# r9y9/deepvoice3_pytorch

Measured on AMD Instinct MI355X. Metric: mel-frames/sec/node (train step, deepvoice3_ljspeech), higher is better.
Workload: dtype f16x3

## Files before the change

deepvoice3_pytorch_amd/csrc/conv_gemm_bf16x3.hip:

```cpp
#include "conv_common.h"
#include <math.h>
#include <type_traits>

typedef __bf16 bf16x8 __attribute__((ext_vector_type(8)));
typedef __bf16 bf16x2 __attribute__((ext_vector_type(2)));
typedef _Float16 f16x8 __attribute__((ext_vector_type(8)));
typedef _Float16 f16x2 __attribute__((ext_vector_type(2)));
typedef float f32x2 __attribute__((ext_vector_type(2)));


namespace {

constexpr int BKC = 32;
constexpr int KB = 4;
constexpr int HALO_MAX = 64;

__device__ __forceinline__ void split8(const float (&v)[8], bf16x8& hi, bf16x8& lo) {
#pragma unroll
  for (int i = 0; i < 8; i += 2) {
    const f32x2 f = {v[i], v[i + 1]};
    const bf16x2 h = __builtin_convertvector(f, bf16x2);
    const f32x2 r = f - __builtin_convertvector(h, f32x2);
    const bf16x2 l = __builtin_convertvector(r, bf16x2);
    hi[i] = h[0]; hi[i + 1] = h[1];
// ... 560 lines not shown
      const bool f16 = a.d.split_terms == DV3_SPLIT_F16X3, m = a.d.xmask != nullptr;
      if (f16) return m ? launch_x3_m<2, 2, 1, true, 3, 1, false, true, 2>(a, lds, st) : launch_x3_m<2, 2, 1, false, 3, 1, false, true, 2>(a, lds, st);
      return m ? launch_x3_m<2, 2, 1, true, 3, 1, false, false, 2>(a, lds, st) : launch_x3_m<2, 2, 1, false, 3, 1, false, false, 2>(a, lds, st);
    }
  }
  if (a.d.split_terms == DV3_SPLIT_F16X3)
    return a.d.xmask ? launch_x3_m<WM, WN, NI, true, 3, 1, false, true>(a, lds, st) : launch_x3_m<WM, WN, NI, false, 3, 1, false, true>(a, lds, st);
  if (a.d.split_terms == 1)
    return a.d.xmask ? launch_x3_m<WM, WN, NI, true, 1>(a, lds, st) : launch_x3_m<WM, WN, NI, false, 1>(a, lds, st);
  return a.d.xmask ? launch_x3_m<WM, WN, NI, true, 3>(a, lds, st) : launch_x3_m<WM, WN, NI, false, 3>(a, lds, st);
}

const TileCfg* pick_tile_x3(const dv3_conv_desc* d, bool gated, int want_tile) {
  const TileCfg* best = nullptr;
  double best_cost = 0;
  const int64_t ntot = (int64_t)d->B * d->Tout;
  for (const TileCfg& c : kCfgs) {
    if (want_tile && c.id != want_tile) continue;
    if (d->pg && !(c.id == 1 || c.id == 2 || c.id == 8 || c.id == 9)) continue;
    const int BM = c.wm * c.mi * 64, BMH = c.wm * c.mi * 32, BN = c.wn * c.ni * 32;
    const int64_t mt = gated ? dv3_cdiv(d->Cg, BMH) : dv3_cdiv(d->M, BM);
    const int64_t ntl = dv3_cdiv64(ntot, BN);
    const double slots = c.id > 6 ? 256.0 : 512.0;
    const double blocks = (double)mt * ntl;
    const double full = floor(blocks / slots), rem = blocks - slots * full;
    const double rounds = (full + (rem == 0 ? 0.0 : (c.id <= 6 && rem <= 256 ? 0.6 : 1.0))) * (slots / 512.0);
    static const double kRel[10] = {0, 1.0, 1.12, 2.0, 2.2, 1.8, 2.0, 9.9, 0.93, 0.87};
    constexpr int kRel2Percent = 112, kRel8Percent = 86;
    double rel = c.id == 2 ? kRel2Percent * 0.01 : c.id == 8 ? kRel8Percent * 0.01 : kRel[c.id];
    if (d->J == 1 && d->Cin <= 512 && (c.id == 1 || c.id == 2 || c.id == 8 || c.id == 9)) rel = 1.0;
    const double cost = rounds * BM * BN * rel;
    if (!best || cost < best_cost) {
      best = &c;
      best_cost = cost;
    }
  }
  return best;
}

}

int dv3_conv_gemm_pp2_dispatch(const dv3_conv_desc* d, hipStream_t st);

int dv3_conv_gemm_bf16x3_dispatch(const dv3_conv_desc* d, hipStream_t st) {
  const bool gated = d->mode == DV3_EPI_GLU || d->mode == DV3_EPI_HIGHWAY;
  if (d->a_bs != 0 || (d->lda & 3) || d->Tin != d->Tout) return 1;
  if ((d->J - 1) * d->dil > HALO_MAX || d->J * 2 > 32) return 1;
  if ((int64_t)d->B * d->Tout >= (1ll << 30) || (int64_t)d->B * d->x_bs >= (1ll << 30)) return 1;
  if (d->xmask && (int64_t)d->B * d->Cin * d->xmask_rs >= (1ll << 30)) return 1;
  if ((int64_t)d->J * ((d->Cin + 31) / 32 * 4) * d->lda >= (1ll << 27)) return 1;
  const int64_t pp2_tiles = (int64_t)(gated ? dv3_cdiv(d->Cg, 128) : dv3_cdiv(d->M, 256)) * dv3_cdiv64((int64_t)d->B * d->Tout, 256);
  const int pp2_min = dv3_sw(DV3_SW_X3_PP2_MIN_TILES), pp2_sk = dv3_sw(DV3_SW_PP2_SK);
  constexpr int kPp2SkUnitsPerCu = 8;
  const bool sk_fill = d->sk_ws && pp2_sk && (d->mode != DV3_EPI_DGRAD || pp2_sk >= 2) && pp2_min > 0 && pp2_tiles * (d->Cin / 32) >= (int64_t)kPp2SkUnitsPerCu * 256;
  if (d->tile_hint == 30 || (pp2_min > 0 && d->tile_hint == 0 && (pp2_tiles >= pp2_min || sk_fill))) {
    const int rc = dv3_conv_gemm_pp2_dispatch(d, st);
    if (rc != 1) return rc;
    if (d->tile_hint == 30) return 1;
  }
  const TileCfg* best = pick_tile_x3(d, gated, d->tile_hint > 20 ? d->tile_hint - 20 : 0);
  if (!best) return 1;
  constexpr int kKsMaxBlocks = 256, kKsMinSteps = 8;
  bool ks_ok = false;
  const int ks_form = dv3_sw(DV3_SW_X3_KS);
  if (ks_form && d->split_terms != 1 && (d->tile_hint == 0 || d->tile_hint == 22)) {
    const int64_t nb2 = (int64_t)(gated ? dv3_cdiv(d->Cg, 64) : dv3_cdiv(d->M, 128)) * dv3_cdiv64((int64_t)d->B * d->Tout, 64);
    const int nch = (d->Cin + 31) / 32;
    const int ksteps = nch * d->J;
    ks_ok = nch >= 2 && (ks_form == 2 || (ksteps >= kKsMinSteps && nb2 <= (ksteps >= 16 ? kKsMaxBlocks : kKsMaxBlocks * 5 / 8)));
    if (ks_ok && d->tile_hint == 0 && (best->id == 4 || best->id == 6)) best = &kCfgs[1];
  }
  const int BM = best->wm * best->mi * 64, BMH = best->wm * best->mi * 32, BN = best->wn * best->ni * 32;
  const int BNH = BN + (d->J - 1) * d->dil;
  const size_t lds = (size_t)(2 * 2 * KB * BM + 2 * 2 * KB * BNH) * 16;
  if (lds > 160 * 1024) return 1;
  ConvArgs a;
  a.d = *d;
  a.a_scalar = 0;
  a.wide = dv3_sw(DV3_SW_X3_WIDE);
  a.prio = dv3_sw(DV3_SW_X3_PRIO);
  a.range_ctr = d->split_terms == DV3_SPLIT_F16X3 ? dv3_range_ctr() : nullptr;
  a.kp = (d->Cin + 31) / 32 * 32;
  a.m_tiles = gated ? dv3_cdiv(d->Cg, BMH) : dv3_cdiv(d->M, BM);
  a.n_tiles = (int)dv3_cdiv64((int64_t)d->B * d->Tout, BN);
  const int64_t nb = (int64_t)a.m_tiles * a.n_tiles;
  DV3_REQUIRE(nb < (1ll << 31), "conv_gemm: grid too large");
  a.n_blocks = (int)nb;
  a.ks = (ks_ok && best->id == 2 && 2 * lds <= 160 * 1024) ? 2 : 0;
  g_dv3_last_conv = (d->split_terms == 1 ? 4000 : d->split_terms == DV3_SPLIT_F16X3 ? 5000 : 3000) + best->id * 10 +
                    ((best->id >= 8 && dv3_sw(DV3_SW_X3_PINGPONG)) ? 1 : 0) + (a.ks == 2 ? 2 : 0);
  if (d->pg) {
    if (d->xmask || d->split_terms == DV3_SPLIT_F16X3 || d->split_terms == 1) return 1;
    g_dv3_last_conv += 600;
    switch (best->id) {
      case 1: return launch_x3_m<2, 2, 2, false, 3, 1, false, false, 1, true>(a, lds, st);
      case 2: return a.ks == 2 ? launch_x3_m<2, 2, 1, false, 3, 1, false, false, 2, true>(a, lds, st)
                               : launch_x3_m<2, 2, 1, false, 3, 1, false, false, 1, true>(a, lds, st);
      case 8: return launch_x3_m<4, 2, 2, false, 3, 1, true, false, 1, true>(a, lds, st);
      case 9: return launch_x3_m<2, 4, 2, false, 3, 1, true, false, 1, true>(a, lds, st);
    }
    return 1;
  }
  switch (best->id) {
    case 1: return launch_x3<2, 2, 2>(a, lds, st);
    case 2: return launch_x3<2, 2, 1>(a, lds, st);
    case 3: return launch_x3<4, 1, 1>(a, lds, st);
    case 4: return launch_x3<2, 1, 1>(a, lds, st);
    case 5: return launch_x3<1, 2, 2>(a, lds, st);
// ... 22 lines not shown
```

deepvoice3_pytorch_amd/csrc/conv_gemm_pp2.hip:

```cpp
#include "conv_common.h"
#include <math.h>
#include <type_traits>

typedef __bf16 bf16x8 __attribute__((ext_vector_type(8)));
typedef __bf16 bf16x2 __attribute__((ext_vector_type(2)));
typedef _Float16 f16x8 __attribute__((ext_vector_type(8)));
typedef float f32x2 __attribute__((ext_vector_type(2)));

namespace {

constexpr int BKC = 32, KB = 4, HALO_MAX = 64;
constexpr int BM = 256, BMH = 128, BN = 256, NT = 512, MI = 2, NI = 2, WN = 4;
constexpr int JT = 3;
constexpr int AU = KB * BM / NT;
constexpr int XI = (KB * (BN + HALO_MAX) + NT - 1) / NT;
static_assert(AU == 2, "one panel unit per k16 phase");

__device__ __forceinline__ void pp2_split8(const float (&v)[8], bf16x8& hi, bf16x8& lo) {
#pragma unroll
  for (int i = 0; i < 8; i += 2) {
    const f32x2 f = {v[i], v[i + 1]};
    const bf16x2 h = __builtin_convertvector(f, bf16x2);
    const f32x2 r = f - __builtin_convertvector(h, f32x2);
    const bf16x2 l = __builtin_convertvector(r, bf16x2);
    hi[i] = h[0]; hi[i + 1] = h[1];
    lo[i] = l[0]; lo[i + 1] = l[1];
  }
}
template <bool F16>
__device__ __forceinline__ f32x16 pp2_mma(const bf16x8& a, const bf16x8& b, const f32x16& c) {
  if constexpr (F16)
    return __builtin_amdgcn_mfma_f32_32x32x16_f16(__builtin_bit_cast(f16x8, a), __builtin_bit_cast(f16x8, b), c, 0, 0, 0);
  else
    return __builtin_amdgcn_mfma_f32_32x32x16_bf16(a, b, c, 0, 0, 0);
}
template <bool OPAQUE>
__device__ __forceinline__ const ConvArgs* dv3_opaque_args(const ConvArgs* a) {
  if constexpr (OPAQUE) {
    int off = 0;
    asm volatile("" : "+s"(off));
    return reinterpret_cast<const ConvArgs*>(reinterpret_cast<const char*>(a) + off);
  } else {
    return a;
  }
}
template <typename T>
__device__ __forceinline__ T pp2_ldg(const void* base, uint32_t byte_off) {
  return *reinterpret_cast<const T*>(reinterpret_cast<const char*>(base) + byte_off);
}

template <bool MASK, bool F16, bool SK = false, int ORD = 0, bool PW = false, bool FG = false>
__global__ __launch_bounds__(NT) void conv_gemm_pp2_kernel(const ConvArgs args) {
  static_assert(!PW || (!MASK && !F16 && !SK), "pair words: the unmasked bf16-pair tile-per-workgroup form");
  static_assert(!FG || (!MASK && !F16 && !SK), "fused gate backward: the unmasked bf16-pair tile-per-workgroup form");
  const dv3_conv_desc& p = args.d;
  extern __shared__ __attribute__((aligned(16))) unsigned char smem_raw[];
  constexpr int J = JT;
  bf16x8* const As = reinterpret_cast<bf16x8*>(smem_raw);
  bf16x8* const Xs = As + 2 * 2 * KB * BM;

  int pid_ = dv3_xcd_remap(blockIdx.x, args.n_blocks);
  if constexpr (SK) {
    const int q = 1 << args.sk_qshift;
    pid_ = (pid_ & ~(q - 1)) + (q - 1 - (pid_ & (q - 1)));
  }
  const int pid = pid_;
  const int nchunks = p.Cin / BKC;
  int seg_u = 0, seg_end = 0, sk_base = 0, sk_rem = 0, sk_g0 = 0;
  if constexpr (SK) {
    const int grp = pid >> args.sk_qshift, slot = pid & ((1 << args.sk_qshift) - 1);
    const bool big = grp < args.sk_tr;
    sk_base = big ? args.sk_base : args.sk_base2;
    sk_rem = big ? args.sk_rem : args.sk_rem2;
    sk_g0 = (grp * args.sk_tg + min(grp, args.sk_tr)) << args.sk_shift;
    seg_u = sk_g0 + slot * sk_base + min(slot, sk_rem);
    seg_end = seg_u + sk_base + (slot < sk_rem ? 1 : 0);
  }
  constexpr bool WIDE_GLU = (ORD & 32) != 0;
  int tid_ = threadIdx.x;
  const int wave_s = __builtin_amdgcn_readfirstlane(tid_ >> 6);
  do {
  const ConvArgs& A = *dv3_opaque_args<SK>(&args);
  const dv3_conv_desc& p = A.d;
  const int dil = p.dil;
  const int BNH = BN + (J - 1) * dil;
  const int xbuf = 2 * KB * BNH;
  if constexpr (SK) {
    int lane_;
    asm volatile("v_mbcnt_lo_u32_b32 %0, -1, 0\n\tv_mbcnt_hi_u32_b32 %0, -1, %0" : "=v"(lane_));
    tid_ = wave_s * 64 + lane_;
  }
  const int tid = tid_;
  const int lane = tid & 63;
  const int wave = __builtin_amdgcn_readfirstlane(tid >> 6);
  const int wm = wave / WN, wn = wave % WN;
  const int l31 = lane & 31, lhi = lane >> 5;
  int tile_ = pid, c0_ = 0, c1_ = nchunks;
  if constexpr (SK) {
    tile_ = seg_u >> A.sk_shift;
    c0_ = seg_u - tile_ * nchunks;
    c1_ = min(nchunks, c0_ + (seg_end - seg_u));
  }
  const int tile = tile_, c0 = SK ? c0_ : 0, c1 = SK ? c1_ : nchunks;
  const int mt = SK ? (tile & (A.m_tiles - 1)) : tile % A.m_tiles;
  const int nt = SK ? (tile >> A.sk_mshift) : tile / A.m_tiles;
  const int n0 = nt * BN;

  const bool gated = (p.mode == DV3_EPI_GLU || p.mode == DV3_EPI_HIGHWAY);
  int h0b, h1b;
  if (gated) {
    h0b = mt * BMH; h1b = p.a_half + mt * BMH;
  } else {
    h0b = mt * BM; h1b = mt * BM + BMH;
  }

  const int Cin = p.Cin, T = p.Tout, lda = p.lda, B = p.B;
  const int Ntot = B * T;
  const int k8_total = A.kp >> 3;
  const bf16x8* __restrict__ Wh = reinterpret_cast<const bf16x8*>(p.a_split);
  const int64_t plane = (int64_t)J * k8_total * lda;
  const float xscale = F16 ? (float)(1 << DV3_F16_ACT_SHIFT) : 1.0f;
  const float dscale = p.drop_scale * xscale;

  uint32_t vbits = 0;
#pragma unroll
  for (int ni = 0; ni < NI; ++ni) {
    const int n = n0 + wn * (NI * 32) + ni * 32 + l31;
    const int bc = n / T, tc = n - bc * T;
    for (int j = 0; j < J; ++j) {
      const int ts = tc + j * dil - p.padL;
      if (n < Ntot && ts >= 0 && ts < T) vbits |= 1u << (j * NI + ni);
    }
  }
  uint32_t need = 0;
  for (int j = 0; j < J; ++j) {
    const uint32_t all = ((1u << NI) - 1u) << (j * NI);
    if (!__all((vbits & all) == all)) need |= 1u << j;
  }
  need = __builtin_amdgcn_readfirstlane(need);

  uint32_t xoff[XI];
  const int n_items = KB * BNH;
  const uint32_t x_rsb = (uint32_t)p.x_rs * 4u;
  const uint32_t c8p = (uint32_t)((Cin + 31) / 32 * 4);
#pragma unroll
  for (int i = 0; i < XI; ++i) {
    const int idx = tid + i * NT;
    const int k8 = idx / BNH, q = idx - k8 * BNH;
    const int f = n0 - p.padL + q;
    int bf = 0, tf = 0;
    if (idx < n_items && f >= 0 && f < Ntot) {
      bf = f / T;
      tf = f - bf * T;
    }
    const int xk8 = k8 < KB ? k8 * 8 : 0;
    xoff[i] = ((uint32_t)bf * (uint32_t)p.x_bs + (uint32_t)tf) * 4u + (uint32_t)xk8 * x_rsb;
  }
  constexpr bool LEAN = (ORD & 2) != 0 && !SK;
  uint32_t aoff_r[2] = {0u, 0u};
  auto aoff_of = [&](int u) -> uint32_t {
    if constexpr (LEAN) return aoff_r[u];
    int t_ = tid;
    asm volatile("" : "+v"(t_));
    const int idx = t_ + u * NT;
    const int col = idx % BM, k8 = idx / BM;
    const bool hi_half = col >= BMH;
    const int gcol = (hi_half ? h1b : h0b) + (col - (hi_half ? BMH : 0));
    return (uint32_t)(k8 * lda + (gcol < lda ? gcol : 0)) * 16u;
  };

  if constexpr (LEAN) {
#pragma unroll
    for (int u = 0; u < 2; ++u) {
      const int idx = tid + u * NT;
      const int col = idx % BM, k8 = idx / BM;
      const bool hi_half = col >= BMH;
      const int gcol = (hi_half ? h1b : h0b) + (col - (hi_half ? BMH : 0));
      aoff_r[u] = (uint32_t)(k8 * lda + (gcol < lda ? gcol : 0)) * 16u;
    }
  }

  bf16x8 ra[2];
  float rx[XI][8];
  uint32_t rk[MASK ? XI : 1];

  auto load_A_unit = [&](int chunk, int j, auto uc) {
    constexpr int u = decltype(uc)::value;
    const bf16x8* srch = Wh + (int64_t)(j * k8_total + chunk * KB) * lda;
    const uint32_t ao = aoff_of(u);
    ra[0] = pp2_ldg<bf16x8>(srch, ao);
    ra[1] = pp2_ldg<bf16x8>(srch + plane, ao);
  };
  auto write_A_unit = [&](int buf, auto uc) {
    constexpr int u = decltype(uc)::value;
    bf16x8* dst = As + buf * (2 * KB * BM);
    dst[tid + u * NT] = ra[0];
    dst[KB * BM + tid + u * NT] = ra[1];
  };
  auto load_X_half = [&](int chunk, auto ic, auto hc) {
    constexpr int i = decltype(ic)::value, h = decltype(hc)::value;
    const char* xb = reinterpret_cast<const char*>(p.x) + (int64_t)(chunk * BKC) * x_rsb;
    uint32_t rs = x_rsb;
    asm volatile("" : "+s"(rs));
#pragma unroll
    for (int e = 4 * h; e < 4 * h + 4; ++e) {
      uint32_t er = (uint32_t)e * rs;
      if constexpr (SK) {
        if (e == 0) { er = 0; asm volatile("" : "+s"(er)); }
      }
      rx[i][e] = pp2_ldg<float>(xb, xoff[i] + er);
    }
    if constexpr (MASK && h == 1) {
      int t_ = tid;
      asm volatile("" : "+v"(t_));
      const int idx = t_ + i * NT;
      const int k8 = idx / BNH, q = idx - k8 * BNH;
      const int f = n0 - p.padL + q;
      int bf = 0, tf = 0;
      if (idx < n_items && f >= 0 && f < Ntot) {
        bf = f / T;
        tf = f - bf * T;
      }
      const uint32_t mo = ((uint32_t)bf * c8p + (uint32_t)(k8 < KB ? k8 : 0)) * (uint32_t)T + (uint32_t)tf;
      rk[i] = (uint32_t)pp2_ldg<uint8_t>(p.xmask_c8 + (int64_t)chunk * 4 * T, mo);
    }
  };
  auto write_X_item = [&](int buf, auto ic) {
    constexpr int i = decltype(ic)::value;
    bf16x8* dst = Xs + buf * xbuf;
    const int idx = tid + i * NT;
    float v[8];
    uint32_t keep = MASK ? rk[i] : 0u;
    if constexpr (MASK && SK) asm("" : "+v"(keep));
#pragma unroll
    for (int e = 0; e < 8; ++e) {
      v[e] = rx[i][e];
      if constexpr (MASK) v[e] *= ((keep >> e) & 1u) ? dscale : 0.f;
      else if (F16) v[e] *= xscale;
    }
    bf16x8 hi, lo;
    if constexpr (PW) {
      uint32_t w[8];
#pragma unroll
      for (int e = 0; e < 8; ++e) w[e] = __float_as_uint(rx[i][e]);
      dv3_pair_units(w, hi, lo);
    } else if constexpr (F16 && LEAN) {
      const float m0 = fmaxf(fmaxf(fabsf(v[0]), fabsf(v[1])), fabsf(v[2]));
      const float m1 = fmaxf(fmaxf(fabsf(v[3]), fabsf(v[4])), fabsf(v[5]));
      const float m = fmaxf(fmaxf(m0, m1), fmaxf(fabsf(v[6]), fabsf(v[7])));
      const bool bad = !(m <= 65504.f);
      if (__builtin_expect(__any(bad), 0)) {
        dv3_note_range(A.range_ctr, dv3_split8_f16(v, hi, lo));
      } else {
        f16x8 h8, l8;
#pragma unroll
        for (int e = 0; e < 8; e += 2) {
          const f32x2 f = {v[e], v[e + 1]};
          typedef _Float16 f16x2_ __attribute__((ext_vector_type(2)));
          const f16x2_ h = __builtin_convertvector(f, f16x2_);
          h8[e] = h[0]; h8[e + 1] = h[1];
          if constexpr ((ORD & 8) != 0) {
            uint32_t l2 = 0u;
            const uint32_t h2 = __builtin_bit_cast(uint32_t, h);
            asm("v_fma_mixlo_f16 %0, %1, -1.0, %2 op_sel:[0,0,0] op_sel_hi:[1,0,0]" : "+v"(l2) : "v"(h2), "v"(v[e]));
            asm("v_fma_mixhi_f16 %0, %1, -1.0, %2 op_sel:[1,0,0] op_sel_hi:[1,0,0]" : "+v"(l2) : "v"(h2), "v"(v[e + 1]));
            const f16x2_ l = __builtin_bit_cast(f16x2_, l2);
            l8[e] = l[0]; l8[e + 1] = l[1];
          } else {
            l8[e] = (_Float16)(v[e] - (float)h[0]);
            l8[e + 1] = (_Float16)(v[e + 1] - (float)h[1]);
          }
        }
        hi = __builtin_bit_cast(bf16x8, h8);
        lo = __builtin_bit_cast(bf16x8, l8);
      }
    } else if constexpr (F16) dv3_note_range(A.range_ctr, dv3_split8_f16(v, hi, lo)); else pp2_split8(v, hi, lo);
    if (idx < n_items) {
      dst[idx] = hi;
      dst[KB * BNH + idx] = lo;
    }
  };
  uint32_t sbad = 0;
  auto write_X_item_nb = [&](int buf, auto ic) {
    constexpr int i = decltype(ic)::value;
    bf16x8* dst = Xs + buf * xbuf;
    const int idx = tid + i * NT;
    float v[8];
    const uint32_t keep = MASK ? rk[i] : 0u;
#pragma unroll
    for (int e = 0; e < 8; ++e) {
      v[e] = rx[i][e];
      if constexpr (MASK) {
        v[e] *= ((keep >> e) & 1u) ? dscale : 0.f;
        asm("" : "+v"(v[e]));
      } else if (F16) v[e] *= xscale;
    }
    bf16x8 hi, lo;
    if constexpr (PW) {
      uint32_t w[8];
#pragma unroll
      for (int e = 0; e < 8; ++e) w[e] = __float_as_uint(rx[i][e]);
      dv3_pair_units(w, hi, lo);
    } else if constexpr (F16) {
      const bool bad = dv3_split8_f16(v, hi, lo);
      sbad += (uint32_t)__builtin_popcountll(__ballot(bad));
    } else {
      pp2_split8(v, hi, lo);
    }
    const int spare = 2 * xbuf - buf * xbuf;
    const bool live = i < 2 || idx < n_items;
    dst[live ? idx : spare] = hi;
    dst[live ? KB * BNH + idx : spare + 1] = lo;
  };
  using U0 = std::integral_constant<int, 0>;
  using U1 = std::integral_constant<int, 1>;
  using U2 = std::integral_constant<int, 2>;
  constexpr bool CVC = (ORD & 64) != 0 && !SK;
  static_assert(XI == 3 && JT == 3, "three activation items per thread, one per tap's pair of k16 phases");

  f32x16 acc[MI][2][NI];
  float zero_ = 0.f;
  if constexpr (SK) asm volatile("" : "+v"(zero_));
#pragma unroll
  for (int mi = 0; mi < MI; ++mi)
#pragma unroll
    for (int h = 0; h < 2; ++h)
#pragma unroll
      for (int ni = 0; ni < NI; ++ni)
#pragma unroll
        for (int r = 0; r < 16; ++r) acc[mi][h][ni][r] = zero_;

  const int a_off = wm * (MI * 32) + l31;
  const int x_off = wn * (NI * 32) + l31;

  load_A_unit(c0, 0, U0{});
  write_A_unit(0, U0{});
  load_A_unit(c0, 0, U1{});
  load_X_half(c0, U0{}, U0{}); load_X_half(c0, U0{}, U1{});
  load_X_half(c0, U1{}, U0{}); load_X_half(c0, U1{}, U1{});
  load_X_half(c0, U2{}, U0{}); load_X_half(c0, U2{}, U1{});
  write_A_unit(0, U1{});
  write_X_item(0, U0{});
  write_X_item(0, U1{});
  write_X_item(0, U2{});
  __syncthreads();
  {
    const int cp = min(c0 + 1, c1 - 1);
    load_A_unit(c0, 1, U0{});
    load_X_half(cp, U0{}, U0{});
    load_X_half(cp, U0{}, U1{});
    load_X_half(cp, U1{}, U0{}); load_X_half(cp, U1{}, U1{});
    load_X_half(cp, U2{}, U0{});
    if constexpr (!CVC) load_X_half(cp, U2{}, U1{});
  }

  const bool pf_on = (ORD & 4) != 0 && !SK && gated && p.r != nullptr;
  const int late = wave >> 2;
  if (late) __syncthreads();
  for (int c = c0; c < c1; ++c) {
    const int cr = c - c0;
    const bf16x8* XsH = Xs + (cr & 1) * xbuf;
    const bf16x8* XsL = XsH + KB * BNH;
    const int cx = min(c + 2, c1 - 1);
    const bool last_chunk = c + 1 == c1;
#pragma unroll
    for (int q = 0; q < 2 * JT; ++q) {
      constexpr int dummy = 0; (void)dummy;
      const int j = q >> 1, s = q & 1;
      const int cur = (cr * JT + j) & 1;
      const bf16x8* AsH = As + cur * (2 * KB * BM);
      const bf16x8* AsL = AsH + KB * BM;
      const bool fix = (need >> j) & 1u;
      bf16x8 ah[MI][2], al[MI][2], bh[NI], bl[NI];
      auto read_frags = [&](bool do_a, bool do_b) {
        const int k8 = 2 * s + lhi;
        if (do_a) {
          const int ai = k8 * BM + a_off;
#pragma unroll
          for (int mi = 0; mi < MI; ++mi) {
            ah[mi][0] = AsH[ai + mi * 32];
            ah[mi][1] = AsH[ai + mi * 32 + BMH];
            al[mi][0] = AsL[ai + mi * 32];
            al[mi][1] = AsL[ai + mi * 32 + BMH];
          }
        }
        if (do_b) {
          const int xi = k8 * BNH + x_off + j * dil;
#pragma unroll
          for (int ni = 0; ni < NI; ++ni) {
            bh[ni] = XsH[xi + ni * 32];
            bl[ni] = XsL[xi + ni * 32];
          }
        }
      };
      auto fix_frags = [&]() {
        const int k8 = 2 * s + lhi; (void)k8;
        if (fix) {
          const bf16x8 zero8 = {0, 0, 0, 0, 0, 0, 0, 0};
#pragma unroll
          for (int ni = 0; ni < NI; ++ni) {
            const bool ok = (vbits >> (j * NI + ni)) & 1u;
            bh[ni] = ok ? bh[ni] : zero8;
            bl[ni] = ok ? bl[ni] : zero8;
          }
        }
      };
      if constexpr ((ORD & 1) != 0) {
        read_frags(true, (ORD & 16) == 0);
        __builtin_amdgcn_sched_barrier(0);
      }
      {
        int jn = j + 1, cn = c;
        if (jn >= JT) { jn = 0; cn = c + 1; }
        int j2 = jn + 1, c2 = cn;
        if (j2 >= JT) { j2 = 0; c2 = cn + 1; }
        if (cn >= c1) { cn = c; jn = j; }
        if (c2 >= c1) { c2 = c; j2 = j; }
        if (s == 0) {
          write_A_unit(cur ^ 1, U0{});
          load_A_unit(cn, jn, U1{});
        } else {
          write_A_unit(cur ^ 1, U1{});
          load_A_unit(c2, j2, U0{});
        }
        if constexpr (CVC) {
          const int cx1 = min(c + 1, c1 - 1);
          if (q == 0) load_X_half(cx1, U2{}, U1{});
          if (q == 1) load_X_half(cx, U0{}, U0{});
          if (q == 2) load_X_half(cx, U0{}, U1{});
          if (q == 3) load_X_half(cx, U1{}, U0{});
          if (q == 4) load_X_half(cx, U1{}, U1{});
          if (q == 5) load_X_half(cx, U2{}, U0{});
        } else {
        if (q == 0) { write_X_item((cr + 1) & 1, U0{}); load_X_half(cx, U0{}, U0{}); }
        if (q == 1) { load_X_half(cx, U0{}, U1{}); }
        if (q == 2) { write_X_item((cr + 1) & 1, U1{}); load_X_half(cx, U1{}, U0{}); }
        if (q == 3) { load_X_half(cx, U1{}, U1{}); }
        if (q == 4) { write_X_item((cr + 1) & 1, U2{}); load_X_half(cx, U2{}, U0{}); }
        if (q == 5) { load_X_half(cx, U2{}, U1{}); }
        }
        if constexpr ((ORD & 4) != 0 && !SK) {
          if ((q == 1 || q == 3) && last_chunk && pf_on) {
            typedef const __attribute__((address_space(1))) void* gptr;
            typedef __attribute__((address_space(3))) void* lptr;
            unsigned char* strip = smem_raw + (size_t)(2 * 2 * KB * BM + 2 * xbuf) * 16 + wave * 256;
            int t_ = tid;
            asm volatile("" : "+v"(t_));
            const int row = t_ >> 2, col = (t_ & 3) * 64 + (q >> 1) * 32;
            const int ch = min(mt * BMH + row, p.Cg - 1);
            const int n = min(n0 + col, Ntot - 1);
            const int bb = n / T, tt = n - bb * T;
            const uint32_t po = ((uint32_t)bb * (uint32_t)p.r_bs + (uint32_t)ch * (uint32_t)p.r_rs + (uint32_t)tt) * 4u;
            __builtin_amdgcn_global_load_lds((gptr)(reinterpret_cast<const char*>(p.r) + po), (lptr)strip, 4, 0, 0);
          }
        }
      }
      __builtin_amdgcn_sched_barrier(0);
      if constexpr ((ORD & 1) == 0) read_frags(true, true);
      else if constexpr ((ORD & 16) != 0) read_frags(false, true);
      fix_frags();
      __syncthreads();
      __builtin_amdgcn_sched_barrier(0);
#pragma unroll
      for (int mi = 0; mi < MI; ++mi)
#pragma unroll
        for (int ni = 0; ni < NI; ++ni) {
          acc[mi][0][ni] = pp2_mma<F16>(al[mi][0], bh[ni], acc[mi][0][ni]);
          acc[mi][1][ni] = pp2_mma<F16>(al[mi][1], bh[ni], acc[mi][1][ni]);
        }
#pragma unroll
      for (int mi = 0; mi < MI; ++mi)
#pragma unroll
        for (int ni = 0; ni < NI; ++ni) {
          acc[mi][0][ni] = pp2_mma<F16>(ah[mi][0], bl[ni], acc[mi][0][ni]);
          acc[mi][1][ni] = pp2_mma<F16>(ah[mi][1], bl[ni], acc[mi][1][ni]);
        }
#pragma unroll
      for (int mi = 0; mi < MI; ++mi)
#pragma unroll
        for (int ni = 0; ni < NI; ++ni) {
          acc[mi][0][ni] = pp2_mma<F16>(ah[mi][0], bh[ni], acc[mi][0][ni]);
          acc[mi][1][ni] = pp2_mma<F16>(ah[mi][1], bh[ni], acc[mi][1][ni]);
        }
      if constexpr (CVC) {
        if (q == 0) write_X_item_nb((cr + 1) & 1, U0{});
        if (q == 2) write_X_item_nb((cr + 1) & 1, U1{});
        if (q == 4) write_X_item_nb((cr + 1) & 1, U2{});
        if ((q & 1) == 0) {
#pragma unroll
          for (int m = 0; m < 22; ++m) {
            __builtin_amdgcn_sched_group_barrier(0x008, 1, 0);
            __builtin_amdgcn_sched_group_barrier(0x002, 3, 0);
          }
          __builtin_amdgcn_sched_group_barrier(0x008, 1, 0);
          __builtin_amdgcn_sched_group_barrier(0x200, 1, 0);
          __builtin_amdgcn_sched_group_barrier(0x008, 1, 0);
          __builtin_amdgcn_sched_group_barrier(0x200, 1, 0);
        }
      }
      __builtin_amdgcn_sched_barrier(0);
      if (!(last_chunk && q == 2 * JT - 1) || !late) __syncthreads();
    }
  }
  if constexpr (CVC && F16) {
    if (sbad != 0 && lane == 0 && A.range_ctr) atomicAdd(A.range_ctr, sbad);
  }

  bool run_tail = true;
  if constexpr (SK) {
    constexpr int ACC = MI * 2 * NI * 16;
    float* const ws = A.sk_ws;
    int* const flags = A.sk_flags;
    if (c0 != 0) {
      char* dst = reinterpret_cast<char*>(ws) + ((size_t)pid * (ACC * NT) + (size_t)tid * 4) * 4;
#pragma unroll
      for (int mi = 0; mi < MI; ++mi)
#pragma unroll
        for (int h = 0; h < 2; ++h)
#pragma unroll
          for (int ni = 0; ni < NI; ++ni)
#pragma unroll
            for (int r4 = 0; r4 < 4; ++r4) {
              typedef float f32x4_ __attribute__((ext_vector_type(4)));
              const f32x4_ v4 = {acc[mi][h][ni][r4 * 4], acc[mi][h][ni][r4 * 4 + 1], acc[mi][h][ni][r4 * 4 + 2], acc[mi][h][ni][r4 * 4 + 3]};
              const char* d4 = dst + (size_t)((((mi * 2 + h) * NI + ni) * 4 + r4) * NT) * 16;
              asm volatile("global_store_dwordx4 %0, %1, off sc0 sc1" ::"v"(d4), "v"(v4) : "memory");
            }
      asm volatile("s_waitcnt vmcnt(0)" ::: "memory");
      __builtin_amdgcn_fence(__ATOMIC_RELEASE, "workgroup");
      __syncthreads();
      if (tid == 0) __hip_atomic_store(flags + pid, 1, __ATOMIC_RELAXED, __HIP_MEMORY_SCOPE_AGENT);
      run_tail = false;
    } else if (c1 < nchunks) {
      const int qm = (1 << A.sk_qshift) - 1;
      for (int w2 = pid + 1; (w2 & qm) != 0; ++w2) {
        const int s2 = sk_g0 + (w2 & qm) * sk_base + min(w2 & qm, sk_rem);
        if (s2 >= (tile + 1) * nchunks) break;
        if (tid == 0)
          while (__hip_atomic_load(flags + w2, __ATOMIC_RELAXED, __HIP_MEMORY_SCOPE_AGENT) == 0) __builtin_amdgcn_s_sleep(8);
        __syncthreads();
        __builtin_amdgcn_fence(__ATOMIC_ACQUIRE, "workgroup");
        const char* src = reinterpret_cast<const char*>(ws) + ((size_t)w2 * (ACC * NT) + (size_t)tid * 4) * 4;
        typedef const __attribute__((address_space(1))) void* gptr_;
        typedef __attribute__((address_space(3))) void* lptr_;
#pragma unroll
        for (int half = 0; half < 2; ++half) {
#pragma unroll
          for (int jq = 0; jq < 16; ++jq) {
            const int qg = half * 16 + jq;
            __builtin_amdgcn_global_load_lds((gptr_)(src + (size_t)(qg * NT) * 16), (lptr_)(smem_raw + (jq * NT + wave * 64) * 16), 16, 0, 17);
          }
          asm volatile("s_waitcnt vmcnt(0)" ::: "memory");
#pragma unroll
          for (int jq = 0; jq < 16; ++jq) {
// ... 38 lines not shown
      bcol[ni] = n / T;
      tcol[ni] = n - bcol[ni] * T;
    }
    if constexpr (FG) {
      const int nw0 = n0e + wn * (NI * 32);
      if (dv3_wide_gate_ok(pt, AT.wide)) {
        float* wl = reinterpret_cast<float*>(smem_raw) + wave * (DV3_WIDE_LDS / 4);
#pragma unroll
        for (int mi = 0; mi < MI; ++mi) {
          const int row0 = wm * (MI * 32) + mi * 32;
          conv_epilogue_wide_block_gate<BM, BMH>(pt, acc[mi][0], mt, row0, 0, lane, nw0, Ntot, wl);
          conv_epilogue_wide_block_gate<BM, BMH>(pt, acc[mi][1], mt, row0, 1, lane, nw0, Ntot, wl);
        }
      } else {
        conv_epilogue_dgrad_gate<BM, BMH, NI>(pt, acc[0], mt, wm * (MI * 32), lhi, l31, bcol, tcol, okc, nw0 >> 5);
        conv_epilogue_dgrad_gate<BM, BMH, NI>(pt, acc[1], mt, wm * (MI * 32) + 32, lhi, l31, bcol, tcol, okc, nw0 >> 5);
      }
    } else
    if (dv3_wide_epilogue_ok(pt, AT.wide)) {
      float* wl = reinterpret_cast<float*>(smem_raw) + wave * (DV3_WIDE_LDS / 4);
      const int nw0 = n0e + wn * (NI * 32);
#pragma unroll
      for (int mi = 0; mi < MI; ++mi) {
        const int row0 = wm * (MI * 32) + mi * 32;
        conv_epilogue_wide_block<BM, BMH>(pt, acc[mi][0], mt, row0, 0, lane, nw0, Ntot, wl);
        conv_epilogue_wide_block<BM, BMH>(pt, acc[mi][1], mt, row0, 1, lane, nw0, Ntot, wl);
      }
    } else if (WIDE_GLU && dv3_wide_glu_ok(pt)) {
      const int nw0 = n0e + wn * (NI * 32);
      conv_epilogue_glu_wide<BMH, NI>(pt, acc[0], mt, wm * (MI * 32), lane, nw0, Ntot);
      conv_epilogue_glu_wide<BMH, NI>(pt, acc[1], mt, wm * (MI * 32) + 32, lane, nw0, Ntot);
    } else {
      bool interior = false;
      if constexpr (!SK)
        interior = AT.fast_tail && gated && !pt.spk && pt.store_mode == DV3_STORE_BCT &&
                   mt * BMH + wm * (MI * 32) + MI * 32 <= pt.Cg && n0e + wn * (NI * 32) + NI * 32 <= Ntot;
      if (!SK && interior) {
        conv_epilogue_glu_interior<BMH, NI>(pt, acc[0], mt, wm * (MI * 32), lhi, bcol, tcol);
        conv_epilogue_glu_interior<BMH, NI>(pt, acc[1], mt, wm * (MI * 32) + 32, lhi, bcol, tcol);
      } else {
        conv_epilogue<BM, BMH, NI, false>(pt, acc[0], gated, mt, wm * (MI * 32), lhi, bcol, tcol, okc);
        conv_epilogue<BM, BMH, NI, false>(pt, acc[1], gated, mt, wm * (MI * 32) + 32, lhi, bcol, tcol, okc);
      }
    }
  }
  if constexpr (SK) {
    seg_u += c1 - c0;
    __syncthreads();
  }
  } while (SK && seg_u < seg_end);
}

#ifndef DV3_PP2_ISA_ONLY
template <bool MASK, bool F16, bool SK = false, int ORD = 0, bool PW = false, bool FG = false>
int launch_pp2(const ConvArgs& a, size_t lds, hipStream_t st) {
  if ((ORD & 4) != 0 && lds + 8 * 256 > 160 * 1024) return launch_pp2<MASK, F16, SK, (ORD & ~4), PW, FG>(a, lds, st);
  static bool attr_set = false;
  if (!attr_set) {
    hipError_t e = hipFuncSetAttribute((const void*)conv_gemm_pp2_kernel<MASK, F16, SK, ORD, PW, FG>,
                                       hipFuncAttributeMaxDynamicSharedMemorySize, 160 * 1024);
    if (e != hipSuccess) {
      dv3_set_error("conv_gemm_pp2: hipFuncSetAttribute: %s", hipGetErrorString(e));
      return DV3_ELAUNCH;
    }
    attr_set = true;
  }
  if ((ORD & 4) != 0) lds += 8 * 256;
  else if ((ORD & 64) != 0) lds += 32;
  hipLaunchKernelGGL((conv_gemm_pp2_kernel<MASK, F16, SK, ORD, PW, FG>), dim3(a.n_blocks), dim3(NT), lds, st, a);
  return dv3_check_launch("conv_gemm_pp2");
}

#endif
}

#ifndef DV3_PP2_ISA_ONLY

constexpr int kSkOverheadChunks = 2, kSkGainPercent = 80;
static int pp2_cu_count() {
  static int n = 0;
  if (!n) {
    int dev = 0, v = 0;
    if (hipGetDevice(&dev) == hipSuccess && hipDeviceGetAttribute(&v, hipDeviceAttributeMultiprocessorCount, dev) == hipSuccess && v > 0) n = v;
    else n = 256;
  }
  return n;
}
int64_t dv3_pp2_sk_ws_bytes() { return (int64_t)pp2_cu_count() * (128 * NT * 4 + 64); }
extern "C" int dv3_conv_streamk_ws_bytes(void) { return (int)dv3_pp2_sk_ws_bytes(); }

int dv3_conv_gemm_pp2_dispatch(const dv3_conv_desc* d, hipStream_t st) {
  if (d->split_terms == 1 || !d->a_split) return 1;
  if (d->xmask && !d->xmask_c8) return 1;
  if (d->J != JT || (d->J - 1) * d->dil > HALO_MAX || (d->Cin & 31)) return 1;
  if (d->a_bs != 0 || (d->lda & 3) || d->Tin != d->Tout) return 1;
  const bool gated = d->mode == DV3_EPI_GLU || d->mode == DV3_EPI_HIGHWAY;
  const bool f16 = d->split_terms == DV3_SPLIT_F16X3;
  const int BNH = BN + (d->J - 1) * d->dil;
  const size_t lds = (size_t)(2 * 2 * KB * BM + 2 * 2 * KB * BNH) * 16;
  if (lds > 160 * 1024) return 1;
  ConvArgs a;
  a.d = *d;
  a.a_scalar = 0;
  a.wide = dv3_sw(DV3_SW_X3_WIDE);
  a.fast_tail = dv3_sw(DV3_SW_PP2_FAST_TAIL);
  a.range_ctr = f16 ? dv3_range_ctr() : nullptr;
  a.kp = (d->Cin + 31) / 32 * 32;
  a.m_tiles = gated ? dv3_cdiv(d->Cg, BMH) : dv3_cdiv(d->M, BM);
  a.n_tiles = (int)dv3_cdiv64((int64_t)d->B * d->Tout, BN);
  const int64_t nb = (int64_t)a.m_tiles * a.n_tiles;
  DV3_REQUIRE(nb < (1ll << 31), "conv_gemm: grid too large");
  a.n_blocks = (int)nb;
  g_dv3_last_conv = (f16 ? 5000 : 3000) + 100 + 1;
  const bool mask = d->xmask_c8 != nullptr;
  if (d->x_pair || d->pg) {
    if (mask || f16) return 1;
    g_dv3_last_conv += (d->x_pair ? 5 : 0) + (d->pg ? 10 : 0);
    if (d->pg) return d->x_pair ? launch_pp2<false, false, false, 81, true, true>(a, lds, st)
                                : launch_pp2<false, false, false, 81, false, true>(a, lds, st);
    return launch_pp2<false, false, false, 81, true>(a, lds, st);
  }
  {
    const int P = pp2_cu_count(), S = d->Cin / BKC;
    const int64_t units = nb * S;
    const int sk_form = dv3_sw(DV3_SW_PP2_SK);
    const int64_t dp = dv3_cdiv64(nb, P) * S, sk = dv3_cdiv64(units, P) + kSkOverheadChunks;
    const bool ws_ok = d->sk_ws && d->sk_ws_bytes >= dv3_pp2_sk_ws_bytes() && units < (1ll << 30);
    const bool dir_ok = d->mode != DV3_EPI_DGRAD || sk_form >= 2;
    const int q = P / 8;
    const bool grp_ok = (P % 8) == 0 && q > 0 && (q & (q - 1)) == 0 && nb >= 8;
    if (ws_ok && dir_ok && grp_ok && sk_form && (S & (S - 1)) == 0 && (a.m_tiles & (a.m_tiles - 1)) == 0 && units >= 2 * P && (sk_form == 2 || sk * 100 < dp * kSkGainPercent)) {
      a.sk_units = (int)units;
      a.sk_tg = (int)(nb / 8);
      a.sk_tr = (int)(nb % 8);
      a.sk_qshift = __builtin_ctz((unsigned)q);
      const int64_t ub = (int64_t)(a.sk_tg + 1) * S, us = (int64_t)a.sk_tg * S;
      a.sk_base = (int)(ub / q);
      a.sk_rem = (int)(ub % q);
      a.sk_base2 = (int)(us / q);
      a.sk_rem2 = (int)(us % q);
      a.sk_shift = __builtin_ctz((unsigned)S);
      a.sk_mshift = __builtin_ctz((unsigned)a.m_tiles);
      a.n_blocks = P;
      a.sk_flags = reinterpret_cast<int*>(d->sk_ws);
      a.sk_ws = reinterpret_cast<float*>(reinterpret_cast<char*>(d->sk_ws) + (size_t)P * 64);
      g_dv3_last_conv += 1;
      const size_t lds_sk = lds;
      if (f16) return mask ? launch_pp2<true, true, true>(a, lds_sk, st) : launch_pp2<false, true, true>(a, lds_sk, st);
      return mask ? launch_pp2<true, false, true>(a, lds_sk, st) : launch_pp2<false, false, true>(a, lds_sk, st);
    }
  }
  {
    const int o = mask ? (f16 ? dv3_sw(DV3_SW_PP2_ORD_M) : 0) : dv3_sw(DV3_SW_PP2_ORD_U);
#define DV3_PP2_ORD_SHIP(oo) \
    if (o == oo) { \
      if (f16) return mask ? launch_pp2<true, true, false, oo>(a, lds, st) : launch_pp2<false, true, false, oo>(a, lds, st); \
      return mask ? launch_pp2<true, false, false, oo>(a, lds, st) : launch_pp2<false, false, false, oo>(a, lds, st); \
    }
    DV3_PP2_ORD_SHIP(17) DV3_PP2_ORD_SHIP(81)
#undef DV3_PP2_ORD_SHIP
  }
  if (f16) return mask ? launch_pp2<true, true>(a, lds, st) : launch_pp2<false, true>(a, lds, st);
  return mask ? launch_pp2<true, false>(a, lds, st) : launch_pp2<false, false>(a, lds, st);
}
#else
namespace {
template __global__ void conv_gemm_pp2_kernel<DV3_PP2_ISA_MASK, true, false, DV3_PP2_ISA_ORD>(const ConvArgs);
// ... 3 lines not shown
```

Baseline: 3.767 million.

## Extend pp2 256x256 conv GEMM kernel to single-tap (1x1) convolutions

Adds a JN template parameter so the large-tile pp2 split-precision GEMM kernel can run one-tap convolutions. Channel counts that are not multiples of 32 are handled by zero-filling the K tail. The activation pipeline is restructured to two items per thread with a separate schedule, and an FMA-based lo-term split is used on the masked bf16 path. The dispatcher routes J==1 convs to pp2 using a tile-count and K-step rule, which adds kernel variants and risks poor occupancy on small shapes.

```diff
diff --git a/deepvoice3_pytorch_amd/csrc/conv_gemm_bf16x3.hip b/deepvoice3_pytorch_amd/csrc/conv_gemm_bf16x3.hip
--- a/deepvoice3_pytorch_amd/csrc/conv_gemm_bf16x3.hip
+++ b/deepvoice3_pytorch_amd/csrc/conv_gemm_bf16x3.hip
@@ -636,8 +636,18 @@
   const int64_t pp2_tiles = (int64_t)(gated ? dv3_cdiv(d->Cg, 128) : dv3_cdiv(d->M, 256)) * dv3_cdiv64((int64_t)d->B * d->Tout, 256);
   const int pp2_min = dv3_sw(DV3_SW_X3_PP2_MIN_TILES), pp2_sk = dv3_sw(DV3_SW_PP2_SK);
   constexpr int kPp2SkUnitsPerCu = 8;
-  const bool sk_fill = d->sk_ws && pp2_sk && (d->mode != DV3_EPI_DGRAD || pp2_sk >= 2) && pp2_min > 0 && pp2_tiles * (d->Cin / 32) >= (int64_t)kPp2SkUnitsPerCu * 256;
-  if (d->tile_hint == 30 || (pp2_min > 0 && d->tile_hint == 0 && (pp2_tiles >= pp2_min || sk_fill))) {
+  const bool sk_fill = d->J != 1 && d->sk_ws && pp2_sk && (d->mode != DV3_EPI_DGRAD || pp2_sk >= 2) && pp2_min > 0 && pp2_tiles * (d->Cin / 32) >= (int64_t)kPp2SkUnitsPerCu * 256;
+  constexpr int kJ1MinTiles = 192, kJ1FwdMinKsteps = 8, kJ1DgradMinKsteps = 4, kJ1CuCount = 256;
+  bool pp2_rule = pp2_min > 0 && (pp2_tiles >= pp2_min || sk_fill);
+  if (d->J == 1) {
+    const bool dgrad = d->mode == DV3_EPI_DGRAD;
+    const int ksteps = (d->Cin + 31) / 32;
+    const int fwd_k = kJ1FwdMinKsteps * (pp2_tiles > kJ1CuCount ? 2 : 1);
+    const bool measured = pp2_tiles >= kJ1MinTiles && ksteps >= (dgrad ? kJ1DgradMinKsteps : fwd_k) &&
+                          2 * dv3_cdiv(d->M, 256) == dv3_cdiv(d->M, 128);
+    pp2_rule = pp2_min == 1 || (pp2_min > 0 && measured);
+  }
+  if (d->tile_hint == 30 || (d->tile_hint == 0 && pp2_rule)) {
     const int rc = dv3_conv_gemm_pp2_dispatch(d, st);
     if (rc != 1) return rc;
     if (d->tile_hint == 30) return 1;
diff --git a/deepvoice3_pytorch_amd/csrc/conv_gemm_pp2.hip b/deepvoice3_pytorch_amd/csrc/conv_gemm_pp2.hip
--- a/deepvoice3_pytorch_amd/csrc/conv_gemm_pp2.hip
+++ b/deepvoice3_pytorch_amd/csrc/conv_gemm_pp2.hip
@@ -13,7 +13,8 @@
 constexpr int BM = 256, BMH = 128, BN = 256, NT = 512, MI = 2, NI = 2, WN = 4;
 constexpr int JT = 3;
 constexpr int AU = KB * BM / NT;
-constexpr int XI = (KB * (BN + HALO_MAX) + NT - 1) / NT;
+constexpr int XI3 = (KB * (BN + HALO_MAX) + NT - 1) / NT;
+constexpr int XI1 = KB * BN / NT;
 static_assert(AU == 2, "one panel unit per k16 phase");
 
 __device__ __forceinline__ void pp2_split8(const float (&v)[8], bf16x8& hi, bf16x8& lo) {
@@ -49,13 +50,15 @@
   return *reinterpret_cast<const T*>(reinterpret_cast<const char*>(base) + byte_off);
 }
 
-template <bool MASK, bool F16, bool SK = false, int ORD = 0, bool PW = false, bool FG = false>
+template <bool MASK, bool F16, bool SK = false, int ORD = 0, bool PW = false, bool FG = false, int JN = JT>
 __global__ __launch_bounds__(NT) void conv_gemm_pp2_kernel(const ConvArgs args) {
   static_assert(!PW || (!MASK && !F16 && !SK), "pair words: the unmasked bf16-pair tile-per-workgroup form");
   static_assert(!FG || (!MASK && !F16 && !SK), "fused gate backward: the unmasked bf16-pair tile-per-workgroup form");
+  static_assert(JN == JT || (JN == 1 && !SK && !FG && (ORD & (4 | 32)) == 0), "one tap: tile per workgroup, plain tails");
+  constexpr int XI = JN == 1 ? XI1 : XI3;
   const dv3_conv_desc& p = args.d;
   extern __shared__ __attribute__((aligned(16))) unsigned char smem_raw[];
-  constexpr int J = JT;
+  constexpr int J = JN;
   bf16x8* const As = reinterpret_cast<bf16x8*>(smem_raw);
   bf16x8* const Xs = As + 2 * 2 * KB * BM;
 
@@ -65,7 +68,7 @@
     pid_ = (pid_ & ~(q - 1)) + (q - 1 - (pid_ & (q - 1)));
   }
   const int pid = pid_;
-  const int nchunks = p.Cin / BKC;
+  const int nchunks = JN == 1 ? (p.Cin + BKC - 1) / BKC : p.Cin / BKC;
   int seg_u = 0, seg_end = 0, sk_base = 0, sk_rem = 0, sk_g0 = 0;
   if constexpr (SK) {
     const int grp = pid >> args.sk_qshift, slot = pid & ((1 << args.sk_qshift) - 1);
@@ -83,7 +86,7 @@
   const ConvArgs& A = *dv3_opaque_args<SK>(&args);
   const dv3_conv_desc& p = A.d;
   const int dil = p.dil;
-  const int BNH = BN + (J - 1) * dil;
+  const int BNH = JN == 1 ? BN : BN + (J - 1) * dil;
   const int xbuf = 2 * KB * BNH;
   if constexpr (SK) {
     int lane_;
@@ -106,7 +109,7 @@
   const int nt = SK ? (tile >> A.sk_mshift) : tile / A.m_tiles;
   const int n0 = nt * BN;
 
-  const bool gated = (p.mode == DV3_EPI_GLU || p.mode == DV3_EPI_HIGHWAY);
+  const bool gated = JN == 3 && (p.mode == DV3_EPI_GLU || p.mode == DV3_EPI_HIGHWAY);
   int h0b, h1b;
   if (gated) {
     h0b = mt * BMH; h1b = p.a_half + mt * BMH;
@@ -202,9 +205,15 @@
     const char* xb = reinterpret_cast<const char*>(p.x) + (int64_t)(chunk * BKC) * x_rsb;
     uint32_t rs = x_rsb;
     asm volatile("" : "+s"(rs));
+    int lim = BKC, kr = 0;
+    if constexpr (JN == 1) {
+      lim = Cin - chunk * BKC;
+      kr = (2 * i + (wave >> 2)) * 8;
+    }
 #pragma unroll
     for (int e = 4 * h; e < 4 * h + 4; ++e) {
       uint32_t er = (uint32_t)e * rs;
+      if constexpr (JN == 1) er = kr + e < lim ? er : 0u - (uint32_t)kr * rs;
       if constexpr (SK) {
         if (e == 0) { er = 0; asm volatile("" : "+s"(er)); }
       }
@@ -225,10 +234,15 @@
       rk[i] = (uint32_t)pp2_ldg<uint8_t>(p.xmask_c8 + (int64_t)chunk * 4 * T, mo);
     }
   };
-  auto write_X_item = [&](int buf, auto ic) {
+  auto write_X_item = [&](int buf, int cw, auto ic) {
     constexpr int i = decltype(ic)::value;
     bf16x8* dst = Xs + buf * xbuf;
     const int idx = tid + i * NT;
+    if constexpr (JN == 1) {
+      const int lim = Cin - cw * BKC, kr = (2 * i + (wave >> 2)) * 8;
+#pragma unroll
+      for (int e = 0; e < 8; ++e) rx[i][e] = kr + e < lim ? rx[i][e] : 0.f;
+    }
     float v[8];
     uint32_t keep = MASK ? rk[i] : 0u;
     if constexpr (MASK && SK) asm("" : "+v"(keep));
@@ -239,6 +253,14 @@
       else if (F16) v[e] *= xscale;
     }
     bf16x8 hi, lo;
+    if constexpr (JN == 1 && MASK && !F16) {
+#pragma unroll
+      for (int e = 0; e < 8; ++e) {
+        const __bf16 h = (__bf16)v[e];
+        hi[e] = h;
+        lo[e] = (__bf16)__builtin_fmaf(rx[i][e], ((keep >> e) & 1u) ? dscale : 0.f, -(float)h);
+      }
+    } else
     if constexpr (PW) {
       uint32_t w[8];
 #pragma unroll
@@ -281,21 +303,38 @@
     }
   };
   uint32_t sbad = 0;
-  auto write_X_item_nb = [&](int buf, auto ic) {
+  auto write_X_item_nb = [&](int buf, int cw, auto ic) {
     constexpr int i = decltype(ic)::value;
     bf16x8* dst = Xs + buf * xbuf;
     const int idx = tid + i * NT;
+    if constexpr (JN == 1) {
+      const int lim = Cin - cw * BKC, kr = (2 * i + (wave >> 2)) * 8;
+#pragma unroll
+      for (int e = 0; e < 8; ++e) rx[i][e] = kr + e < lim ? rx[i][e] : 0.f;
+    }
     float v[8];
     const uint32_t keep = MASK ? rk[i] : 0u;
+    constexpr bool FMA_LO = JN == 1 && MASK && !F16;
+    float ksel[FMA_LO ? 8 : 1];
 #pragma unroll
     for (int e = 0; e < 8; ++e) {
       v[e] = rx[i][e];
       if constexpr (MASK) {
-        v[e] *= ((keep >> e) & 1u) ? dscale : 0.f;
+        const float sel = ((keep >> e) & 1u) ? dscale : 0.f;
+        v[e] *= sel;
         asm("" : "+v"(v[e]));
+        if constexpr (FMA_LO) ksel[e] = sel;
       } else if (F16) v[e] *= xscale;
     }
     bf16x8 hi, lo;
+    if constexpr (FMA_LO) {
+#pragma unroll
+      for (int e = 0; e < 8; ++e) {
+        const __bf16 h = (__bf16)v[e];
+        hi[e] = h;
+        lo[e] = (__bf16)__builtin_fmaf(rx[i][e], ksel[e], -(float)h);
+      }
+    } else
     if constexpr (PW) {
       uint32_t w[8];
 #pragma unroll
@@ -316,7 +355,7 @@
   using U1 = std::integral_constant<int, 1>;
   using U2 = std::integral_constant<int, 2>;
   constexpr bool CVC = (ORD & 64) != 0 && !SK;
-  static_assert(XI == 3 && JT == 3, "three activation items per thread, one per tap's pair of k16 phases");
+  static_assert((XI == 3 && JN == 3) || (XI == 2 && JN == 1), "three taps: one activation item per tap's pair of k16 phases; one tap: one per phase");
 
   f32x16 acc[MI][2][NI];
   float zero_ = 0.f;
@@ -338,20 +377,26 @@
   load_A_unit(c0, 0, U1{});
   load_X_half(c0, U0{}, U0{}); load_X_half(c0, U0{}, U1{});
   load_X_half(c0, U1{}, U0{}); load_X_half(c0, U1{}, U1{});
-  load_X_half(c0, U2{}, U0{}); load_X_half(c0, U2{}, U1{});
+  if constexpr (JN == 3) { load_X_half(c0, U2{}, U0{}); load_X_half(c0, U2{}, U1{}); }
   write_A_unit(0, U1{});
-  write_X_item(0, U0{});
-  write_X_item(0, U1{});
-  write_X_item(0, U2{});
+  write_X_item(0, c0, U0{});
+  write_X_item(0, c0, U1{});
+  if constexpr (JN == 3) write_X_item(0, c0, U2{});
   __syncthreads();
   {
     const int cp = min(c0 + 1, c1 - 1);
+    if constexpr (JN == 3) {
     load_A_unit(c0, 1, U0{});
     load_X_half(cp, U0{}, U0{});
     load_X_half(cp, U0{}, U1{});
     load_X_half(cp, U1{}, U0{}); load_X_half(cp, U1{}, U1{});
     load_X_half(cp, U2{}, U0{});
     if constexpr (!CVC) load_X_half(cp, U2{}, U1{});
+    } else {
+      load_A_unit(cp, 0, U0{});
+      load_X_half(cp, U0{}, U0{}); load_X_half(cp, U0{}, U1{});
+      load_X_half(cp, U1{}, U0{}); load_X_half(cp, U1{}, U1{});
+    }
   }
 
   const bool pf_on = (ORD & 4) != 0 && !SK && gated && p.r != nullptr;
@@ -364,10 +409,10 @@
     const int cx = min(c + 2, c1 - 1);
     const bool last_chunk = c + 1 == c1;
 #pragma unroll
-    for (int q = 0; q < 2 * JT; ++q) {
+    for (int q = 0; q < 2 * J; ++q) {
       constexpr int dummy = 0; (void)dummy;
       const int j = q >> 1, s = q & 1;
-      const int cur = (cr * JT + j) & 1;
+      const int cur = (cr * J + j) & 1;
       const bf16x8* AsH = As + cur * (2 * KB * BM);
       const bf16x8* AsL = AsH + KB * BM;
       const bool fix = (need >> j) & 1u;
@@ -411,9 +456,9 @@
       }
       {
         int jn = j + 1, cn = c;
-        if (jn >= JT) { jn = 0; cn = c + 1; }
+        if (jn >= J) { jn = 0; cn = c + 1; }
         int j2 = jn + 1, c2 = cn;
-        if (j2 >= JT) { j2 = 0; c2 = cn + 1; }
+        if (j2 >= J) { j2 = 0; c2 = cn + 1; }
         if (cn >= c1) { cn = c; jn = j; }
         if (c2 >= c1) { c2 = c; j2 = j; }
         if (s == 0) {
@@ -423,6 +468,18 @@
           write_A_unit(cur ^ 1, U1{});
           load_A_unit(c2, j2, U0{});
         }
+        if constexpr (JN == 1) {
+          if constexpr (CVC) {
+            if (q == 1) {
+              load_X_half(cx, U0{}, U0{}); load_X_half(cx, U0{}, U1{});
+              load_X_half(cx, U1{}, U0{}); load_X_half(cx, U1{}, U1{});
+            }
+          } else {
+            const int cw = min(c + 1, c1 - 1);
+            if (q == 0) { write_X_item((cr + 1) & 1, cw, U0{}); load_X_half(cx, U0{}, U0{}); load_X_half(cx, U0{}, U1{}); }
+            if (q == 1) { write_X_item((cr + 1) & 1, cw, U1{}); load_X_half(cx, U1{}, U0{}); load_X_half(cx, U1{}, U1{}); }
+          }
+        } else
         if constexpr (CVC) {
           const int cx1 = min(c + 1, c1 - 1);
           if (q == 0) load_X_half(cx1, U2{}, U1{});
@@ -432,11 +489,11 @@
           if (q == 4) load_X_half(cx, U1{}, U1{});
           if (q == 5) load_X_half(cx, U2{}, U0{});
         } else {
-        if (q == 0) { write_X_item((cr + 1) & 1, U0{}); load_X_half(cx, U0{}, U0{}); }
+        if (q == 0) { write_X_item((cr + 1) & 1, c, U0{}); load_X_half(cx, U0{}, U0{}); }
         if (q == 1) { load_X_half(cx, U0{}, U1{}); }
-        if (q == 2) { write_X_item((cr + 1) & 1, U1{}); load_X_half(cx, U1{}, U0{}); }
+        if (q == 2) { write_X_item((cr + 1) & 1, c, U1{}); load_X_half(cx, U1{}, U0{}); }
         if (q == 3) { load_X_half(cx, U1{}, U1{}); }
-        if (q == 4) { write_X_item((cr + 1) & 1, U2{}); load_X_half(cx, U2{}, U0{}); }
+        if (q == 4) { write_X_item((cr + 1) & 1, c, U2{}); load_X_half(cx, U2{}, U0{}); }
         if (q == 5) { load_X_half(cx, U2{}, U1{}); }
         }
         if constexpr ((ORD & 4) != 0 && !SK) {
@@ -483,9 +540,25 @@
           acc[mi][1][ni] = pp2_mma<F16>(ah[mi][1], bh[ni], acc[mi][1][ni]);
         }
       if constexpr (CVC) {
-        if (q == 0) write_X_item_nb((cr + 1) & 1, U0{});
-        if (q == 2) write_X_item_nb((cr + 1) & 1, U1{});
-        if (q == 4) write_X_item_nb((cr + 1) & 1, U2{});
+        if constexpr (JN == 1) {
+          if (q == 0) {
+            const int cw = min(c + 1, c1 - 1);
+            write_X_item_nb((cr + 1) & 1, cw, U0{});
+            write_X_item_nb((cr + 1) & 1, cw, U1{});
+#pragma unroll
+            for (int m = 0; m < 22; ++m) {
+              __builtin_amdgcn_sched_group_barrier(0x008, 1, 0);
+              __builtin_amdgcn_sched_group_barrier(0x002, 6, 0);
+            }
+            __builtin_amdgcn_sched_group_barrier(0x008, 1, 0);
+            __builtin_amdgcn_sched_group_barrier(0x200, 2, 0);
+            __builtin_amdgcn_sched_group_barrier(0x008, 1, 0);
+            __builtin_amdgcn_sched_group_barrier(0x200, 2, 0);
+          }
+        } else {
+        if (q == 0) write_X_item_nb((cr + 1) & 1, c, U0{});
+        if (q == 2) write_X_item_nb((cr + 1) & 1, c, U1{});
+        if (q == 4) write_X_item_nb((cr + 1) & 1, c, U2{});
         if ((q & 1) == 0) {
 #pragma unroll
           for (int m = 0; m < 22; ++m) {
@@ -497,9 +570,10 @@
           __builtin_amdgcn_sched_group_barrier(0x008, 1, 0);
           __builtin_amdgcn_sched_group_barrier(0x200, 1, 0);
         }
+        }
       }
       __builtin_amdgcn_sched_barrier(0);
-      if (!(last_chunk && q == 2 * JT - 1) || !late) __syncthreads();
+      if (!(last_chunk && q == 2 * J - 1) || !late) __syncthreads();
     }
   }
   if constexpr (CVC && F16) {
@@ -644,12 +718,12 @@
 }
 
 #ifndef DV3_PP2_ISA_ONLY
-template <bool MASK, bool F16, bool SK = false, int ORD = 0, bool PW = false, bool FG = false>
+template <bool MASK, bool F16, bool SK = false, int ORD = 0, bool PW = false, bool FG = false, int JN = JT>
 int launch_pp2(const ConvArgs& a, size_t lds, hipStream_t st) {
-  if ((ORD & 4) != 0 && lds + 8 * 256 > 160 * 1024) return launch_pp2<MASK, F16, SK, (ORD & ~4), PW, FG>(a, lds, st);
+  if ((ORD & 4) != 0 && lds + 8 * 256 > 160 * 1024) return launch_pp2<MASK, F16, SK, (ORD & ~4), PW, FG, JN>(a, lds, st);
   static bool attr_set = false;
   if (!attr_set) {
-    hipError_t e = hipFuncSetAttribute((const void*)conv_gemm_pp2_kernel<MASK, F16, SK, ORD, PW, FG>,
+    hipError_t e = hipFuncSetAttribute((const void*)conv_gemm_pp2_kernel<MASK, F16, SK, ORD, PW, FG, JN>,
                                        hipFuncAttributeMaxDynamicSharedMemorySize, 160 * 1024);
     if (e != hipSuccess) {
       dv3_set_error("conv_gemm_pp2: hipFuncSetAttribute: %s", hipGetErrorString(e));
@@ -659,7 +733,7 @@
   }
   if ((ORD & 4) != 0) lds += 8 * 256;
   else if ((ORD & 64) != 0) lds += 32;
-  hipLaunchKernelGGL((conv_gemm_pp2_kernel<MASK, F16, SK, ORD, PW, FG>), dim3(a.n_blocks), dim3(NT), lds, st, a);
+  hipLaunchKernelGGL((conv_gemm_pp2_kernel<MASK, F16, SK, ORD, PW, FG, JN>), dim3(a.n_blocks), dim3(NT), lds, st, a);
   return dv3_check_launch("conv_gemm_pp2");
 }
 
@@ -684,9 +758,10 @@
 int dv3_conv_gemm_pp2_dispatch(const dv3_conv_desc* d, hipStream_t st) {
   if (d->split_terms == 1 || !d->a_split) return 1;
   if (d->xmask && !d->xmask_c8) return 1;
-  if (d->J != JT || (d->J - 1) * d->dil > HALO_MAX || (d->Cin & 31)) return 1;
+  const bool one = d->J == 1;
+  const bool gated = d->mode == DV3_EPI_GLU || d->mode == DV3_EPI_HIGHWAY;
+  if (one ? (gated || d->pg || d->padL != 0) : (d->J != JT || (d->J - 1) * d->dil > HALO_MAX || (d->Cin & 31))) return 1;
   if (d->a_bs != 0 || (d->lda & 3) || d->Tin != d->Tout) return 1;
-  const bool gated = d->mode == DV3_EPI_GLU || d->mode == DV3_EPI_HIGHWAY;
   const bool f16 = d->split_terms == DV3_SPLIT_F16X3;
   const int BNH = BN + (d->J - 1) * d->dil;
   const size_t lds = (size_t)(2 * 2 * KB * BM + 2 * 2 * KB * BNH) * 16;
@@ -705,6 +780,15 @@
   a.n_blocks = (int)nb;
   g_dv3_last_conv = (f16 ? 5000 : 3000) + 100 + 1;
   const bool mask = d->xmask_c8 != nullptr;
+  if (one) {
+    if (d->x_pair) {
+      if (mask || f16) return 1;
+      g_dv3_last_conv += 5;
+      return launch_pp2<false, false, false, 81, true, false, 1>(a, lds, st);
+    }
+    if (f16) return mask ? launch_pp2<true, true, false, 81, false, false, 1>(a, lds, st) : launch_pp2<false, true, false, 81, false, false, 1>(a, lds, st);
+    return mask ? launch_pp2<true, false, false, 81, false, false, 1>(a, lds, st) : launch_pp2<false, false, false, 81, false, false, 1>(a, lds, st);
+  }
   if (d->x_pair || d->pg) {
     if (mask || f16) return 1;
     g_dv3_last_conv += (d->x_pair ? 5 : 0) + (d->pg ? 10 : 0);
```

After: 3.779 million (median of 5 runs). No clear change (+0.3%).
